# mhrice/RemFx

Hardware: AMD Instinct MI355X
Metric: audio-seconds/sec fwd+bwd (whole job) (higher is better)
Workload: dtype bf16 (fp32 accumulate); 1 GPU; Hybrid Demucs (cfg/model/demucs.yaml) train step, +exp=chorus_aug model=demucs; clips_per_gpu=64, global_batch=64, clip_samples=262144, parallelism=dp1, rccl_ranks=0, ranks=1, streams=4

## Files before the change

### include/remfx_hip.h

```cpp
#ifndef REMFX_HIP_H
#define REMFX_HIP_H

#include <stdint.h>

#ifdef __cplusplus
extern "C" {
#endif

#define RFX_ABI_VERSION 1

enum rfx_act {
  RFX_ACT_NONE = 0,
  RFX_ACT_RELU = 1,
  RFX_ACT_GELU = 2,
  RFX_ACT_TANH = 3,
  RFX_ACT_PRELU = 4,
  RFX_ACT_LEAKY = 5,
  RFX_ACT_SIGMOID = 6
};

typedef struct rfx_ktab_entry {
  int32_t off;
  int32_t da;
  int32_t db;
// ... 350 lines not shown
  void* cm_out;
  int64_t cm_ns, cm_cs, cm_as;
  int32_t cm_fold;
} rfx_cl_conv_desc;
int rfx_cl_conv(const rfx_cl_conv_desc* d, void* stream);
int rfx_cl_conv_variant(const rfx_cl_conv_desc* d);
int rfx_cl_pack(const float* src, const int32_t* idx, int64_t n, void* dst, void* stream);
int rfx_cl_from_cm(const void* src, int32_t src_bf16, int64_t s_ns, int64_t s_cs, int64_t s_as, int32_t N, int32_t C, int32_t A,
                   int32_t B, const rfx_cl_tensor* dst, const rfx_cl_tensor* res, const rfx_cl_tensor* aux, int32_t mode, void* stream);
int rfx_cl_to_cm(const rfx_cl_tensor* src, int32_t N, int32_t C, int32_t A, int32_t B, void* dst, int32_t dst_bf16, int64_t d_ns,
                 int64_t d_cs, int64_t d_as, const void* aux16, void* stream);
int rfx_cl_im2col_s4(const float* src, int64_t s_ns, int64_t s_cs, int64_t s_as, int32_t N, int32_t Cs, int32_t IA, int32_t IB, int32_t OA,
                     int32_t OB, int32_t along_b, void* dst, void* stream);
int rfx_cl_im2col_fm(const float* src, const float* coef_a, const float* coef_b, int32_t N, int32_t F, int32_t bins, void* dst, void* stream);
int rfx_fm_cm_affine(const float* in, float* out, const float* coef_a, const float* coef_b, int32_t N, int32_t bins, int32_t F, int32_t to_fm,
                     void* stream);
int rfx_cl_dgelu(const void* g, const void* z, void* out, int64_t n, void* stream);
int rfx_cl_dglu(const void* g, const void* zab, void* out, int64_t npos, int32_t C, void* stream);

typedef struct rfx_cl_wgrad_desc {
  rfx_cl_tensor p, q;
  int32_t N, OA, IA, B;
  int32_t SA, da0, NTR;
  int32_t NTC, db0, db_step;
  int32_t M, Cq, CW;
  int32_t RW, WK;
  int32_t S, ahead, bias;
  int32_t PW;
  float* ws;
} rfx_cl_wgrad_desc;
int64_t rfx_cl_wgrad_ws_floats(const rfx_cl_wgrad_desc* d);
int rfx_cl_wgrad(const rfx_cl_wgrad_desc* d, void* stream);
int rfx_cl_wgrad_variant(const rfx_cl_wgrad_desc* d);
int rfx_cl_wgrad_reduce(const float* ws, const int32_t* map, int64_t nmap, int32_t S, int32_t DT, int32_t RW, int32_t WK, float* dw,
                        int64_t wn, float* db, int32_t accumulate, void* stream);

typedef struct rfx_cl_dconv_desc {
  const void* x;
  const void* gy;
  void* y;
  void* a; void* hpre; float* stats;
  void* dz; void* dh; float* partial;
  const void* w1p; const void* w2p; const void* w2dp; const void* w1dp;
  const float *b1, *g1w, *g1b, *b2, *g2w, *g2b, *scale;
  int32_t S, C, H, dil, grid, x_or_gy_ok;
  float eps;
  int32_t TPS;
  float* tsum; float* sums;
  float* pg_dst[5];
} rfx_cl_dconv_desc;
int rfx_cl_dconv_ok(int32_t C, int32_t H, int32_t T, int32_t backward);
int rfx_cl_dconv_fwd(const rfx_cl_dconv_desc* d, void* stream);
int rfx_cl_dconv_bwd(const rfx_cl_dconv_desc* d, float* pgrad, void* stream);

int rfx_cl_rowsum(const rfx_cl_tensor* x, int32_t N, int32_t A, int32_t B, int32_t C, int32_t G, float scale, float* partial, float* out,
                  int32_t accumulate, void* stream);

int rfx_segment_split(const float* x, float* out, int32_t rows, int64_t T, int32_t L, int32_t hop, int32_t S, void* stream);
int rfx_segment_merge(const float* y, float* out, int32_t rows, int64_t T, int32_t L, int32_t hop, int32_t lead, int32_t trail,
                      int32_t S, void* stream);
int rfx_segment_split_c(const float* x, float* out, int32_t B, int32_t C, int64_t T, int32_t L, int32_t hop, int32_t S, void* stream);
int rfx_segment_merge_c(const float* y, float* out, int32_t B, int32_t Co, int64_t T, int32_t L, int32_t hop, int32_t lead, int32_t trail,
                        int32_t S, void* stream);

int rfx_fir_same(const float* x, float* y, const float* x2, float* y2, int32_t R, int64_t L, int64_t x_stride, int64_t y_stride,
                 int64_t x2_stride, int64_t y2_stride, const float* h, int32_t K, int32_t flip, void* stream);
// ... 12 lines not shown
```

### remfx_amd/_lib.py

```python
import ctypes as C
import glob
import os
import subprocess

_HERE = os.path.dirname(os.path.abspath(__file__))
_ROOT = os.path.dirname(_HERE)
CSRC = os.path.join(_HERE, "csrc")
INCLUDE = os.path.join(_ROOT, "include")
LIBDIR = os.path.join(_HERE, "_C")
LIBPATH = os.environ.get("RFX_LIBPATH_DEV") or os.path.join(LIBDIR, "libremfx_hip.so")

HIPCC_FLAGS = ["--offload-arch=gfx950", "-O3", "-std=c++17", "-fPIC", "-ffp-contract=fast",
               "-I" + INCLUDE, "-I" + CSRC]


def sources():
    return sorted(glob.glob(os.path.join(CSRC, "*.hip")))


def _stale():
    if not os.path.exists(LIBPATH):
        return True
    t = os.path.getmtime(LIBPATH)
    deps = sources() + glob.glob(os.path.join(CSRC, "*.h")) + glob.glob(os.path.join(INCLUDE, "*.h"))
# ... 53 lines not shown

class StftDesc(C.Structure):
    _fields_ = [(n, C.c_int32) for n in ("R", "T", "n_fft", "hop", "win", "bins", "frame0", "frames_out",
                                         "mode", "extra_pad_l", "extra_pad_r", "in_mode", "in_offset",
                                         "herm")] + \
               [(n, C.c_float) for n in ("scale", "eps", "alpha")] + [("accum", C.c_int32)]


class ClTensor(C.Structure):
    _fields_ = [("p", C.c_void_p), ("ns", C.c_int64), ("as_", C.c_int64), ("bs", C.c_int32), ("c0", C.c_int32)]


class ClConvDesc(C.Structure):
    _fields_ = [("inp", ClTensor)] + \
               [(n, C.c_int32) for n in ("N", "IA", "IB", "OA", "OB", "SA", "NTR", "NCH", "NTC", "KS", "da0", "da_step", "db0",
                                         "db_step", "wrapb")] + \
               [("apack", C.c_void_p)] + \
               [(n, C.c_int32) for n in ("M", "BM", "mode", "G", "g_off", "OAo", "Co")] + \
               [("bias", C.c_void_p), ("rowadd", C.c_void_p), ("out0", ClTensor), ("out1", ClTensor), ("aux0", ClTensor), ("res", ClTensor),
                ("cm_out", C.c_void_p), ("cm_ns", C.c_int64), ("cm_cs", C.c_int64), ("cm_as", C.c_int64), ("cm_fold", C.c_int32)]


class ClDconvDesc(C.Structure):
    _fields_ = [(n, C.c_void_p) for n in ("x", "gy", "y", "a", "hpre", "stats", "dz", "dh", "partial", "w1p", "w2p", "w2dp", "w1dp",
                                          "b1", "g1w", "g1b", "b2", "g2w", "g2b", "scale")] + \
               [(n, C.c_int32) for n in ("S", "C", "H", "dil", "grid", "x_or_gy_ok")] + [("eps", C.c_float), ("TPS", C.c_int32), ("tsum", C.c_void_p), ("sums", C.c_void_p), ("pg_dst", C.c_void_p * 5)]


class ClWgradDesc(C.Structure):
    _fields_ = [("p", ClTensor), ("q", ClTensor)] + \
               [(n, C.c_int32) for n in ("N", "OA", "IA", "B", "SA", "da0", "NTR", "NTC", "db0", "db_step", "M", "Cq", "CW", "RW", "WK",
                                         "S", "ahead", "bias", "PW")] + \
               [("ws", C.c_void_p)]


_P, _I32, _I64 = C.c_void_p, C.c_int32, C.c_int64
SIGNATURES = {
    "rfx_abi_version": [],
    "rfx_gemm_pick_r": [_I32, _I32],
    "rfx_pack_a": [_P, _P, _I64, _I32, _I32, _I32, _I32, _I32, _P, _P],
    "rfx_unpack_add": [_P, _P, _I64, _I32, _I32, _I32, _P, _I32, _P],
    "rfx_unpack_add_bias": [_P, _P, _I64, _I32, _I32, _I32, _P, _I32, _P, _I32, _P],
    "rfx_unpack_set": [_P, _P, _I64, _I32, _I32, _I32, _P, _I32, _P],
    "rfx_unpack_col": [_P, _I32, _I32, _I32, _I32, _P, _P],
    "rfx_gemm_fwd": [C.POINTER(GemmDesc), _P, _P, _P, _P, C.POINTER(Epilogue), _P, _P, _I32, _I32, _P, _I32, _P],
    "rfx_gemm_fwd_variant": [C.POINTER(GemmDesc), C.POINTER(Epilogue), _I32, _I32],
    "rfx_gemm_wgrad": [C.POINTER(GemmDesc), _P, _P, _P, _P, _I64, C.POINTER(C.c_int32), _I32, _P],
    "rfx_gemm_wgrad_variant": [C.POINTER(GemmDesc), _I64, _I32],
    "rfx_fft_analysis": [C.POINTER(StftDesc), _P, _P, _P, _P, _P],
    "rfx_fft_synthesis_ws": [C.POINTER(StftDesc)],
    "rfx_fft_synthesis": [C.POINTER(StftDesc), _P, _P, _P, _P, _P, _P],
    "rfx_stft_loss_reduce": [_P, _P, _I32, _I64, C.c_float, _P, _P, _P],
    "rfx_stft_loss_grad": [_P, _P, _I32, _I64, C.c_float, _P, C.c_float, C.c_float, _P, _P, _P],
    "rfx_stft_loss_grad_m": [_P, _P, _I32, _I64, C.c_float, _P, C.c_float, C.c_float, _P, _P, _P],
    "rfx_stft_pair_loss_ws": [C.POINTER(StftDesc)],
    "rfx_stft_pair_loss": [C.POINTER(StftDesc), _P, _P, _P, C.c_float, _P, _P, _P, _P, _P],
    "rfx_fft_synthesis_lossgrad": [C.POINTER(StftDesc), _P, _P, _P, C.c_float, C.c_float, C.c_float, _P, _P, _P, _P, _P],
    "rfx_l1_grad": [_P, _P, _I64, C.c_float, _P, _P, _P],
    "rfx_sisdr_sums": [_P, _P, _I32, _I64, _I64, _I64, _P, _P, _P],
    "rfx_sisdr_finish": [_P, _I32, _I64, _I32, C.c_double, _P, _P],
    "rfx_time_sums_ws": [_I32, _I64],
    "rfx_time_sums": [_P, _P, _I32, _I64, _I64, _I64, _I32, C.c_double, C.c_double, C.c_double, _P, _P, _P],
    "rfx_time_loss_rows": [_P, _I32, _I64, _I32, _I32, C.c_double, _I32, _P, _P, _P, _P],
    "rfx_time_loss_grad": [_P, _P, _I32, _I64, _I64, _I64, _P, _I32, C.c_double, C.c_double, C.c_double, _P, _I32, _P, _P],
    "rfx_logcosh_ws": [_I32, _I64],
    "rfx_logcosh_rows": [_P, _P, _I32, _I64, _I64, _I64, C.c_double, C.c_double, _P, _P, _P],
# ... 70 lines not shown
    "rfx_localstate_gen_fwd": [_P, _P, _P, _P, _I32, _I32, _I32, _I32, _I32, _P, _P, _P],
    "rfx_localstate_gen_bwd": [_P, _P, _P, _P, _P, _P, _P, _I32, _I32, _I32, _I32, _I32, _P, _P, _P, _P, _P],
    "rfx_mha_fwd": [_P, _P, _P, _I32, _I32, _I32, _I32, _P, _P, _P],
    "rfx_mha_bwd": [_P, _P, _P, _P, _P, _P, _I32, _I32, _I32, _I32, _P, _P, _P, _P],
    "rfx_localstate_mfma_ok": [_I32, _I32, _I32, _I32, _I32],
    "rfx_localstate_mfma_fwd": [_P, _P, _P, _P, _I32, _I32, _I32, _I32, _I32, _P, _P],
    "rfx_localstate_mfma_bwd": [_P, _P, _P, _P, _P, _I32, _I32, _I32, _I32, _I32, _P, _P, _P, _P, _P, _P],
    "rfx_blstm_frames": [_P, _P, _P, _I32, _I32, _I32, _I32, _I32, _I32, _I32, _P],
    "rfx_span_mask": [_P, _I32, _I32, _I32, _P, _P, _P, _P, _P],
    "rfx_dropout": [_P, _P, _I64, C.c_float, C.c_uint64, _P],
    "rfx_row_moments_slots": [_I64],
    "rfx_row_moments": [_P, _I32, _I64, _P, _P, _P, C.c_float, _P, _P, _P],
    "rfx_row_affine": [_P, _P, _P, _P, _I32, _I64, _P],
    "rfx_row_affine_add": [_P, _P, _P, _P, _P, _I32, _I32, _I64, _P],
    "rfx_fm_cm_affine_g": [_P, _P, _P, _P, _I32, _I32, _I32, _I32, _I32, _P],
    "rfx_lstm_pack_bytes": [_I32],
    "rfx_lstm_pack": [_P, _I32, _P, _P],
    "rfx_lstm_cat_params": [_P, _P, _P, _P, _P, _P, _I32, _I32, _P, _P, _P],
    "rfx_lstm_grad_scatter": [_P, _P, _I32, _I32, _P, _P, _P, _P, _P, _P, _P],
    "rfx_lstm_local": [_I32, _I32, _I32, _I32],
    "rfx_lstm_pack_local": [_P, _I32, _P, _P],
    "rfx_lstm_ws_bytes": [_I32],
    "rfx_lstm_fwd": [_P, _P, _I32, _I32, _I32, _P, _P, _P, _P, _I32, _P],
    "rfx_lstm_bwd": [_P, _P, _P, _P, _I32, _I32, _I32, _P, _P, _I32, _P],
    "rfx_lstm_set_local": [_I32, _I32],
    "rfx_channel_sum_ws": [_P, _I32, _I32, _I32, _I32, _I64, _I64, _I64, _I64],
    "rfx_channel_sum": [_P, _I32, _I32, _I32, _I32, _I64, _I64, _I64, _I64, _P, _P, _P],
    "rfx_cl_conv": [C.POINTER(ClConvDesc), _P],
    "rfx_cl_conv_variant": [C.POINTER(ClConvDesc)],
    "rfx_cl_pack": [_P, _P, _I64, _P, _P],
    "rfx_cl_wgrad_ws_floats": [_P],
    "rfx_cl_wgrad": [_P, _P],
    "rfx_cl_wgrad_variant": [_P],
    "rfx_cl_wgrad_reduce": [_P, _P, _I64, _I32, _I32, _I32, _I32, _P, _I64, _P, _I32, _P],
    "rfx_cl_from_cm": [_P, _I32, _I64, _I64, _I64, _I32, _I32, _I32, _I32, C.POINTER(ClTensor), C.POINTER(ClTensor), C.POINTER(ClTensor),
                       _I32, _P],
    "rfx_cl_rowsum": [C.POINTER(ClTensor), _I32, _I32, _I32, _I32, _I32, C.c_float, _P, _P, _I32, _P],
    "rfx_cl_to_cm": [C.POINTER(ClTensor), _I32, _I32, _I32, _I32, _P, _I32, _I64, _I64, _I64, _P, _P],
    "rfx_cl_dgelu": [_P, _P, _P, _I64, _P],
    "rfx_cl_dglu": [_P, _P, _P, _I64, _I32, _P],
    "rfx_cl_im2col_s4": [_P, _I64, _I64, _I64, _I32, _I32, _I32, _I32, _I32, _I32, _I32, _P, _P],
    "rfx_cl_im2col_fm": [_P, _P, _P, _I32, _I32, _I32, _P, _P],
    "rfx_fm_cm_affine": [_P, _P, _P, _P, _I32, _I32, _I32, _I32, _P],
    "rfx_cl_dconv_ok": [_I32, _I32, _I32, _I32],
    "rfx_cl_dconv_fwd": [_P, _P],
    "rfx_cl_dconv_bwd": [_P, _P, _P],
    "rfx_segment_split": [_P, _P, _I32, _I64, _I32, _I32, _I32, _P],
    "rfx_segment_merge": [_P, _P, _I32, _I64, _I32, _I32, _I32, _I32, _I32, _P],
    "rfx_segment_split_c": [_P, _P, _I32, _I32, _I64, _I32, _I32, _I32, _P],
    "rfx_segment_merge_c": [_P, _P, _I32, _I32, _I64, _I32, _I32, _I32, _I32, _I32, _P],
    "rfx_fir_same": [_P, _P, _P, _P, _I32, _I64, _I64, _I64, _I64, _I64, _P, _I32, _I32, _P],
    "rfx_sum_diff": [_P, _P, _P, _P, _P, _P, _I32, _I64, _I64, _I64, _I64, _I64, _P],
    "rfx_sum_diff_adj": [_P, _P, _P, _I32, _I64, _P],
}

_RET64 = {"rfx_cl_wgrad_ws_floats", "rfx_cplx_slots", "rfx_norm_bwd_work_floats", "rfx_stft_pair_loss_ws", "rfx_stft_scaled_loss_ws", "rfx_channel_sum_ws", "rfx_fft_synthesis_ws",
          "rfx_fx_phaser_ws_floats", "rfx_fx_sox_reverb_ws_floats", "rfx_fx_normalize_ws_bytes", "rfx_time_sums_ws", "rfx_logcosh_ws"}
_lib = None


def lib():
    global _lib
    if _lib is not None:
        return _lib
    import torch
    if not os.path.exists(LIBPATH):
# ... 18 lines not shown
```

### remfx_amd/clast.py

```python
import ctypes as C
import os as _os

import numpy as np
import torch

from . import _lib, ops
from ._lib import ClConvDesc, ClTensor, ClWgradDesc, check

TRACE = None

EPI = {"store": 0, "gelu": 1, "glu": 2, "dgelu": 3, "dglu": 4, "store_cm": 5}


def _stream():
    return C.c_void_p(ops.raw_stream())


def cl_tensor(t, c0=0):
    ct = ClTensor()
    if t is None:
        return ct
    if t.dtype != torch.bfloat16 or t.dim() != 4 or t.stride(3) != 1 or not t.is_cuda:
        raise ValueError(f"channels-last operand must be a 4-D bf16 GPU tensor with dense channels (got {t.dtype}, {tuple(t.shape)}, {t.stride()})")
    ct.p = t.data_ptr()
# ... 303 lines not shown
            if tiles > 16:
                continue
            ctn = -(-Cq // CW)
            cost = (ctn, ctn * CW - Cq)
            if best is None or cost < best[0]:
                best = (cost, CW, tiles)
        if best is None:
            raise ValueError(f"channels-last weight gradient: no tiling for {T} taps x {Cq} channels")
        _, self.CW, tiles = best
        self.WK = 1 if tiles > 8 else (2 if tiles > 4 else 4)
        self.WC = 8 // self.WK
        self.MTn, self.CTn = -(-M // (32 * self.RW)), -(-Cq // self.CW)
        self.DT = self.MTn * self.CTn
        hb = max(abs(db0 + t * db_step) for t in range(NTC))
        self.ahead = None
        for PW, amin in (((128, 2), (64, 1)) if _os.environ.get("RFX_CLW_PW", "128") == "128" else ((64, 1),)):
            NP = PW // 16 * self.RW
            NQ = -(-((PW + 2 * hb) * self.CW * 2) // 1024)
            PPW = -(-(NP + SA * NQ) // 8)
            if PPW > 6 or (PW // 16) % self.WK:
                continue
            for ahead in (4, 3, 2, 1):
                R = -(-(NTR + ahead * SA) // SA) * SA
                if ahead >= amin and (ahead + 1) * NP * 1024 + R * NQ * 1024 <= self.LDS_MAX and (ahead - 1) * PPW <= 24:
                    self.ahead, self.PW = ahead, PW
                    break
            if self.ahead is not None:
                break
        if self.ahead is None:
            raise ValueError("channels-last weight gradient: tile does not fit LDS")
        self.map = self._build_map(widx)
        self._dev = {}

    def _build_map(self, widx):
        RW, NT, WC = self.RW, 2, self.WC
        NCG = self.CW // 16
        HN = self.NTR * self.NTC * NCG
        bias_tile = -(-HN // 2)
        shape = (self.MTn, self.CTn, WC, RW, NT, 16, 64)
        mt, ct, cw, i, t, r, lane = np.meshgrid(*[np.arange(s, dtype=np.int64) for s in shape], indexing="ij", sparse=True)
        m = mt * 32 * RW + 32 * i + (r & 3) + 8 * (r >> 2) + 4 * (lane >> 5)
        l31 = lane & 31
        tile = cw * NT + t
        hh = 2 * tile + (l31 >> 4)
        cgl, tt = hh % NCG, hh // NCG
        tc, tr = tt % self.NTC, tt // self.NTC
        c = ct * self.CW + cgl * 16 + (l31 & 15)
        ok = (hh < HN) & (m < self.M) & (c < self.Cq)
        idx = widx(np.minimum(m, self.M - 1), np.minimum(tr, self.NTR - 1), tc, np.minimum(c, self.Cq - 1))
        out = np.where(np.broadcast_to(ok, shape), np.broadcast_to(idx, shape), -1)
        if self.bias:
            isb = (tile == bias_tile) & (l31 == 0) & (ct == 0) & (m < self.M)
            out = np.where(np.broadcast_to(isb, shape), np.broadcast_to(self.wn + m, shape), out)
        flat = out.reshape(-1)
        used = flat[flat >= 0]
        assert used.size == np.unique(used).size, "weight-gradient map: a destination is written twice"
        return np.ascontiguousarray(flat.astype(np.int32))

    def splits(self, steps):
        S = max(1, min(steps, -(-CLW_SPLITS // self.DT)))
        sps = -(-steps // S)
        return -(-steps // sps)


def _dev_map(form, device):
    key = str(device)
    v = form._dev.get(key)
    if v is None:
        v = torch.from_numpy(form.map).to(device)
        form._dev[key] = v
    return v


def wgrad(form, p, q, N, OA, IA, B, dw, db=None, accumulate=False, p_c0=0, q_c0=0):
    if form.bias and db is None:
        raise ValueError("this weight-gradient form carries the bias gradient: pass db")
    d = ClWgradDesc()
    d.p, d.q = cl_tensor(p, p_c0), cl_tensor(q, q_c0)
    d.N, d.OA, d.IA, d.B = N, OA, IA, B
# ... 54 lines not shown
```

### remfx_amd/csrc/cl_wgrad.hip

```cpp
#include "cl_common.h"

#ifndef RFX_CLW_DBG_BUILD
#define RFX_CLW_DBG_BUILD 0
#endif
#define CLW_DBG RFX_CLW_DBG_BUILD
#include <stdlib.h>

struct ClWgK {
  rfx_cl_wgrad_desc d;
  int32_t nbq, MTn, CTn, DT, spx;
  int32_t total, sps;
  int32_t NP, NQ, TP, PPW;
  int32_t PSLOT, QROWB, QROWP, R, PD, PRE, HB;
  int32_t HN, NCG, bias_tile;
  uint32_t p_bytes, q_bytes;
};

#define CL_WG_MAXP 6

__device__ __forceinline__ void clw_wait_vm(int n) {
  switch (n) {
    case 0: CL_VMCNT(0); break;   case 1: CL_VMCNT(1); break;   case 2: CL_VMCNT(2); break;   case 3: CL_VMCNT(3); break;
    case 4: CL_VMCNT(4); break;   case 5: CL_VMCNT(5); break;   case 6: CL_VMCNT(6); break;   case 7: CL_VMCNT(7); break;
    case 8: CL_VMCNT(8); break;   case 9: CL_VMCNT(9); break;   case 10: CL_VMCNT(10); break; case 11: CL_VMCNT(11); break;
    case 12: CL_VMCNT(12); break; case 13: CL_VMCNT(13); break; case 14: CL_VMCNT(14); break; case 15: CL_VMCNT(15); break;
    case 16: CL_VMCNT(16); break; case 17: CL_VMCNT(17); break; case 18: CL_VMCNT(18); break; case 19: CL_VMCNT(19); break;
    case 20: CL_VMCNT(20); break; case 21: CL_VMCNT(21); break; case 22: CL_VMCNT(22); break; case 23: CL_VMCNT(23); break;
    default: CL_VMCNT(24); break;
  }
}

typedef short clw_s16x4 __attribute__((ext_vector_type(4)));
typedef short clw_s16x8 __attribute__((ext_vector_type(8)));
__device__ __forceinline__ cl_bf16x8 clw_frag(const unsigned char* p, int step4) {
  const clw_s16x4 lo = __builtin_amdgcn_ds_read_tr16_b64_v4i16((__attribute__((address_space(3))) clw_s16x4*)(p));
  const clw_s16x4 hi = __builtin_amdgcn_ds_read_tr16_b64_v4i16((__attribute__((address_space(3))) clw_s16x4*)(p + step4));
  const clw_s16x8 v = {lo[0], lo[1], lo[2], lo[3], hi[0], hi[1], hi[2], hi[3]};
  return __builtin_bit_cast(cl_bf16x8, v);
}

struct ClwIt {
  int n, bq, oa, pre;
};

template <int RW, int WK, int PW>
__global__ __launch_bounds__(512, 2) void cl_wgrad_kernel(const ClWgK g) {
  constexpr int NT = 2, WC = 8 / WK, KSW = (PW / 16) / WK;
  constexpr int PROWB = 64 * RW;
  extern __shared__ __attribute__((aligned(16))) unsigned char clw_smem[];
  const rfx_cl_wgrad_desc& d = g.d;
  const int tid = threadIdx.x;
  const int wave = __builtin_amdgcn_readfirstlane(tid >> 6), lane = tid & 63;
  const int kq = wave / WC, cw = wave % WC;
  const int bid = blockIdx.x, xcd = bid & 7, qx = bid >> 3;
  const bool grouped = d.S >= 8;
  const int dt = grouped ? qx % g.DT : bid % g.DT, split = grouped ? xcd * g.spx + qx / g.DT : bid / g.DT;
  if (split >= d.S) return;
  const int mt = dt / g.CTn, ct = dt - mt * g.CTn;
  const int tau0 = split * g.sps;
  const int tau1 = min(tau0 + g.sps, g.total);
  const int OA = d.OA;

  unsigned char* const pbase_lds = clw_smem;
  unsigned char* const qbase_lds = clw_smem + g.PD * g.PSLOT;

  int32_t rel[CL_WG_MAXP], bpos[CL_WG_MAXP];
  int lds_off[CL_WG_MAXP], prow[CL_WG_MAXP];
#pragma unroll
  for (int i = 0; i < CL_WG_MAXP; ++i) {
    int e = wave + 8 * i;
    e = e < g.TP ? e : g.TP - 1;
    if (e < g.NP) {
      prow[i] = -1;
      lds_off[i] = e * 1024;
      const int o = e * 1024 + lane * 16;
      const int pos = o / PROWB, cb = o - pos * PROWB;
      const bool ok = pos < PW && (mt * 32 * RW + (cb >> 1)) < d.M;
      rel[i] = ok ? (int32_t)((pos * d.p.bs + d.p.c0 + mt * 32 * RW) * 2 + cb) : (int32_t)CL_OOB;
      bpos[i] = 0;
    } else {
      const int qe = e - g.NP;
      const int rr = qe / g.NQ, qi = qe - rr * g.NQ;
      prow[i] = rr;
      lds_off[i] = rr * g.QROWB + qi * 1024;
      const int o = qi * 1024 + lane * 16;
      const int pos = o / g.QROWP, cb = o - pos * g.QROWP;
      const bool ok = pos < PW + 2 * g.HB && (ct * d.CW + (cb >> 1)) < d.Cq;
      rel[i] = ok ? (int32_t)(((pos - g.HB) * d.q.bs + d.q.c0 + ct * d.CW) * 2 + cb) : (int32_t)CL_OOB;
      bpos[i] = ok ? pos - g.HB : 0x40000000;
    }
  }

  const int gq = lane >> 4, i16 = lane & 15;
  const int rowhalf = gq & 1, khalf = gq >> 1, s_e = i16 >> 2, q4 = i16 & 3;
  const uint32_t a0 = (uint32_t)((8 * khalf + s_e) * PROWB + rowhalf * 32 + q4 * 8);
  int rtap[NT];
  uint32_t bconst[NT];
#pragma unroll
  for (int t = 0; t < NT; ++t) {
    int hh = 2 * (cw * NT + t) + rowhalf;
    hh = hh < g.HN ? hh : 0;
    const int cgl = hh % g.NCG, tt = hh / g.NCG;
    const int tc = tt % d.NTC;
    rtap[t] = tt / d.NTC;
    bconst[t] = (uint32_t)((g.HB + d.db0 + tc * d.db_step + 8 * khalf + s_e) * g.QROWP + cgl * 32 + q4 * 8);
  }
  const bool ones_wave = d.bias && g.bias_tile >= 0 && (g.bias_tile / NT) == cw;
  const int ones_t = g.bias_tile % NT;

  f32x16 acc[RW][NT];
#pragma unroll
  for (int i = 0; i < RW; ++i)
#pragma unroll
    for (int t = 0; t < NT; ++t)
#pragma unroll
      for (int r = 0; r < 16; ++r) acc[i][t][r] = 0.f;

  const int col0 = tau0 / OA;
  const int ncols = (tau1 - 1) / OA - col0 + 1;
  const int L = (tau1 - tau0) + g.PRE * ncols;
  ClwIt it_i = {col0 / g.nbq, col0 % g.nbq, tau0 - col0 * OA - g.PRE, g.PRE}, it_c = it_i;
  auto advance = [&](ClwIt& it) {
    ++it.oa;
    if (it.pre > 0) --it.pre;
    if (it.oa == OA) {
      it.oa = -g.PRE; it.pre = g.PRE;
      if (++it.bq == g.nbq) { it.bq = 0; ++it.n; }
    }
  };
  int rs_n = it_i.n;
  cl_i32x4 rs_p = cl_rsrc_words(reinterpret_cast<const uint16_t*>(d.p.p) + (int64_t)rs_n * d.p.ns, g.p_bytes);
  cl_i32x4 rs_q = cl_rsrc_words(reinterpret_cast<const uint16_t*>(d.q.p) + (int64_t)rs_n * d.q.ns, g.q_bytes);
  int iu = 0, wp = 0, ps_i = 0;
  auto issue_next = [&]() {
    if (CLW_DBG & 1) { advance(it_i); ++iu; return; }
    const int b0 = it_i.bq * PW;
    const bool real = it_i.pre == 0;
    if (it_i.n != rs_n) {
// ... 4 lines not shown
    const int32_t pb = (int32_t)(((int64_t)it_i.oa * d.p.as + (int64_t)b0 * d.p.bs) * 2);
    const int ia0 = it_i.oa * d.SA + d.da0 + d.NTR - d.SA;
#pragma unroll
    for (int i = 0; i < CL_WG_MAXP; ++i) {
      if (i < g.PPW) {
        if (prow[i] < 0) {
          const uint32_t vo = real ? (uint32_t)(rel[i] + pb) : CL_OOB;
          cl_glds16_quiet(rs_p, pbase_lds + ps_i * g.PSLOT + lds_off[i], vo);
        } else {
          const int ia = ia0 + prow[i];
          const bool rok = (unsigned)ia < (unsigned)d.IA;
          const int32_t qb = (int32_t)(((int64_t)ia * d.q.as + (int64_t)b0 * d.q.bs) * 2);
          const uint32_t vo = (rok && (unsigned)(b0 + bpos[i]) < (unsigned)d.B) ? (uint32_t)(rel[i] + qb) : CL_OOB;
          cl_glds16_quiet(rs_q, qbase_lds + wp * g.QROWB + lds_off[i], vo);
        }
      }
    }
    wp += d.SA;
    wp = wp >= g.R ? wp - g.R : wp;
    ps_i = ps_i + 1 == g.PD ? 0 : ps_i + 1;
    advance(it_i);
    ++iu;
  };

  int cpm = (d.SA - d.NTR + 2 * g.R) % g.R;
  int ps_c = 0;
  const int ahead = g.PD - 1;
  for (int i = 0; i < ahead; ++i)
    if (iu < L) issue_next();
  const bool late = wave >= 4 && !(CLW_DBG & 16);
  auto frags = [&](int ks, const unsigned char* pb, const unsigned char* const (&qb)[NT], cl_bf16x8 (&af)[RW], cl_bf16x8 (&bf)[NT], int i) {
#pragma unroll
    for (int r = 0; r < RW; ++r)
      af[r] = (CLW_DBG & 2) ? __builtin_bit_cast(cl_bf16x8, make_uint4(lane, r, ks, i)) : clw_frag(pb + ks * 16 * PROWB + r * 64, 4 * PROWB);
#pragma unroll
    for (int t = 0; t < NT; ++t) {
      if (ones_wave && t == ones_t) {
        const clw_s16x8 one = {0x3f80, 0x3f80, 0x3f80, 0x3f80, 0x3f80, 0x3f80, 0x3f80, 0x3f80};
        bf[t] = __builtin_bit_cast(cl_bf16x8, one);
      } else {
        bf[t] = (CLW_DBG & 2) ? __builtin_bit_cast(cl_bf16x8, make_uint4(lane, t, ks, i)) : clw_frag(qb[t] + ks * 16 * g.QROWP, 4 * g.QROWP);
      }
    }
  };
  for (int i = 0; i < L; ++i) {
    const int left = L - 1 - i;
    clw_wait_vm((left < ahead - 1 ? left : ahead - 1) * g.PPW);
    if (!(CLW_DBG & 8)) __builtin_amdgcn_s_barrier();
    __builtin_amdgcn_sched_barrier(0);
    if (!late && iu < L) issue_next();
    __builtin_amdgcn_sched_barrier(0);
    if (it_c.pre == 0 && !(CLW_DBG & 4)) {
      const unsigned char* pb = pbase_lds + ps_c * g.PSLOT + a0;
      const unsigned char* qb[NT];
#pragma unroll
      for (int t = 0; t < NT; ++t) {
        int sl = cpm + rtap[t];
        sl = sl >= g.R ? sl - g.R : sl;
        qb[t] = qbase_lds + sl * g.QROWB + bconst[t];
      }
      cl_bf16x8 af[2][RW], bf[2][NT];
      frags(kq, pb, qb, af[0], bf[0], i);
#pragma unroll
      for (int ksi = 0; ksi < KSW; ++ksi) {
        if (ksi + 1 < KSW) frags(kq + (ksi + 1) * WK, pb, qb, af[(ksi + 1) & 1], bf[(ksi + 1) & 1], i);
#pragma unroll
        for (int r = 0; r < RW; ++r)
#pragma unroll
          for (int t = 0; t < NT; ++t) acc[r][t] = __builtin_amdgcn_mfma_f32_32x32x16_bf16(af[ksi & 1][r], bf[ksi & 1][t], acc[r][t], 0, 0, 0);
      }
    }
    __builtin_amdgcn_sched_barrier(0);
    if (late && iu < L) issue_next();
    cpm += d.SA;
    cpm = cpm >= g.R ? cpm - g.R : cpm;
    ps_c = ps_c + 1 == g.PD ? 0 : ps_c + 1;
    advance(it_c);
  }

  float* wsp = d.ws + ((size_t)((size_t)split * g.DT + dt) * 8 + wave) * (RW * NT * 16 * 64) + lane;
#pragma unroll
  for (int r = 0; r < RW; ++r)
#pragma unroll
    for (int t = 0; t < NT; ++t)
#pragma unroll
      for (int e = 0; e < 16; ++e) wsp[((r * NT + t) * 16 + e) * 64] = acc[r][t][e];
// ... 12 lines not shown
    hb = v < 0 ? (-v > hb ? -v : hb) : (v > hb ? v : hb);
  }
  if (hb > 8) return -1;
  k.d = d;
  k.HB = hb;
  k.nbq = d.B / d.PW;
  k.MTn = (d.M + 32 * d.RW - 1) / (32 * d.RW);
  k.CTn = (d.Cq + d.CW - 1) / d.CW;
  k.DT = k.MTn * k.CTn;
  k.spx = (d.S + 7) / 8;
  const int64_t total = (int64_t)d.N * k.nbq * d.OA;
  if (total >= 0x7fffffffLL) return -1;
  k.total = (int)total;
  k.sps = (int)((total + d.S - 1) / d.S);
  if ((total + k.sps - 1) / k.sps != d.S) return -1;
  k.NCG = d.CW / 16;
  k.HN = d.NTR * d.NTC * k.NCG;
  const int WC = 8 / d.WK, tiles = (k.HN + 1) / 2;
  if (tiles > WC * 2) return -1;
  k.bias_tile = d.bias ? tiles : -1;
  if (d.bias && tiles + 1 > WC * 2) return -1;
  k.NP = (d.PW * 64 * d.RW + 1023) / 1024;
  k.QROWP = d.CW * 2;
  k.NQ = ((d.PW + 2 * hb) * k.QROWP + 1023) / 1024;
  k.TP = k.NP + d.SA * k.NQ;
  k.PPW = (k.TP + 7) / 8;
  if (k.PPW > CL_WG_MAXP) return -1;
  k.PSLOT = k.NP * 1024;
  k.QROWB = k.NQ * 1024;
  k.PRE = (d.NTR - d.SA + d.SA - 1) / d.SA;
  k.PD = d.ahead + 1;
  k.R = ((d.NTR + d.ahead * d.SA + d.SA - 1) / d.SA) * d.SA;
  if ((k.PD - 2) * k.PPW > 24 && k.PD > 2) return -1;
  const int64_t pb = ((int64_t)(d.OA - 1) * d.p.as + (int64_t)d.B * d.p.bs) * 2;
  const int64_t qb = ((int64_t)(d.IA - 1) * d.q.as + (int64_t)d.B * d.q.bs) * 2;
  if (pb <= 0 || qb <= 0 || pb >= 0x7fffffffLL || qb >= 0x7fffffffLL) return -1;
  k.p_bytes = (uint32_t)pb;
  k.q_bytes = (uint32_t)qb;
  return 0;
}

template <int RW, int WK, int PW>
static int clw_launch1(const ClWgK& k, int lds, hipStream_t s, bool query) {
  const bool grouped = k.d.S >= 8;
  if (query) return RW | WK << 2 | PW << 5 | (grouped ? 1 : 0) << 13;
  static int attr_lds = 0;
  if (lds > attr_lds) {
    if (hipFuncSetAttribute(reinterpret_cast<const void*>(&cl_wgrad_kernel<RW, WK, PW>), hipFuncAttributeMaxDynamicSharedMemorySize, lds) !=
        hipSuccess)
      return -3;
    attr_lds = lds;
  }
  hipLaunchKernelGGL((cl_wgrad_kernel<RW, WK, PW>), dim3((unsigned)(grouped ? 8 * k.spx * k.DT : k.d.S * k.DT)), dim3(512), lds, s, k);
  RFX_CHECK_LAUNCH();
  return 0;
}
template <int RW, int WK>
static int clw_launch(const ClWgK& k, int lds, hipStream_t s, bool query) {
  return k.d.PW == 128 ? clw_launch1<RW, WK, 128>(k, lds, s, query) : clw_launch1<RW, WK, 64>(k, lds, s, query);
}

extern "C" int64_t rfx_cl_wgrad_ws_floats(const rfx_cl_wgrad_desc* dp) {
  ClWgK k;
  if (!dp || clw_geometry(*dp, k)) return -1;
  return (int64_t)dp->S * k.DT * 8 * dp->RW * 2 * 1024;
}

static int clw_run(const rfx_cl_wgrad_desc* dp, void* stream, bool query) {
  if (!dp || !dp->p.p || !dp->q.p || !dp->ws) return -1;
  ClWgK k;
  if (clw_geometry(*dp, k)) return -1;
  const int lds = k.PD * k.PSLOT + k.R * k.QROWB;
  if (lds > 160 * 1024) return -1;
  hipStream_t s = (hipStream_t)stream;
  if (dp->RW == 3) {
    if (dp->WK == 1) return clw_launch<3, 1>(k, lds, s, query);
    if (dp->WK == 2) return clw_launch<3, 2>(k, lds, s, query);
    return clw_launch<3, 4>(k, lds, s, query);
  }
  if (dp->WK == 1) return clw_launch<2, 1>(k, lds, s, query);
  if (dp->WK == 2) return clw_launch<2, 2>(k, lds, s, query);
  return clw_launch<2, 4>(k, lds, s, query);
}
extern "C" int rfx_cl_wgrad(const rfx_cl_wgrad_desc* dp, void* stream) { return clw_run(dp, stream, false); }
extern "C" int rfx_cl_wgrad_variant(const rfx_cl_wgrad_desc* dp) { return clw_run(dp, nullptr, true); }

__global__ __launch_bounds__(256) void cl_wgrad_reduce_kernel(const float* __restrict__ ws, const int32_t* __restrict__ map, int64_t nmap,
                                                              int S, int DT, int WC, int WK, int per_wave, float* __restrict__ dw,
                                                              int64_t wn, float* __restrict__ db, int accumulate) {
  __shared__ float part[4][64];
  const int l = threadIdx.x & 63, sg = threadIdx.x >> 6;
  const int64_t e = (int64_t)blockIdx.x * 64 + l;
  const int32_t dst = e < nmap ? map[e] : -1;
  float sum = 0.f;
  if (dst >= 0) {
    const int64_t inner = e % per_wave;
    const int64_t dc = e / per_wave;
    const int cw = (int)(dc % WC);
    const int64_t dt = dc / WC;
    const int nsrc = S * WK;
    const int per = (nsrc + 3) / 4;
    const int i0 = sg * per, i1 = min(i0 + per, nsrc);
    const int64_t sstride = (int64_t)DT * 8 * per_wave;
    const float* base = ws + dt * 8 * per_wave + (int64_t)cw * per_wave + inner;
    auto src = [&](int i) { return base[(int64_t)(i / WK) * sstride + (int64_t)(i % WK) * WC * per_wave]; };
    int i = i0;
    for (; i + 8 <= i1; i += 8) {
      float v[8];
#pragma unroll
      for (int u = 0; u < 8; ++u) v[u] = src(i + u);
#pragma unroll
      for (int u = 0; u < 8; ++u) sum += v[u];
    }
    for (; i < i1; ++i) sum += src(i);
  }
  part[sg][l] = sum;
  __syncthreads();
  if (sg == 0 && dst >= 0) {
// ... 17 lines not shown
```

Measured before the change: 3742 audio-seconds/sec.

## Swizzle wgrad LDS layouts and reorder 48-channel tile enumeration to cut bank conflicts

Changes the LDS layout of the channels-last weight-gradient kernel. P rows are XOR-swizzled for RW=2, and Q rows get a 64-channel XOR swizzle or a blocked 48-channel layout with per-row flipping. A custom half-tile enumeration table is used for CW=48, NTC=3, with the matching host-side map in Python. The aim is fewer LDS bank conflicts in the MFMA fragment loads. A layout query API is added for verification, and the extra address arithmetic plus the Python/device mapping consistency are added risks.

```diff
diff --git a/include/remfx_hip.h b/include/remfx_hip.h
--- a/include/remfx_hip.h
+++ b/include/remfx_hip.h
@@ -406,6 +406,14 @@
 int64_t rfx_cl_wgrad_ws_floats(const rfx_cl_wgrad_desc* d);
 int rfx_cl_wgrad(const rfx_cl_wgrad_desc* d, void* stream);
 int rfx_cl_wgrad_variant(const rfx_cl_wgrad_desc* d);
+typedef struct rfx_cl_wgrad_lane {
+  int32_t a_addr[3][2];
+  int32_t b_addr[2][2], b_half[2], b_cg[2], b_tc[2], b_tr[2], b_row[2];
+  int32_t dma_row, dma_addr, dma_pos, dma_ch, dma_zero;
+  int32_t p_slot_bytes, q_row_bytes, q_rows, pieces, halo;
+} rfx_cl_wgrad_lane;
+int rfx_cl_wgrad_layout(const rfx_cl_wgrad_desc* d, int32_t dt, int32_t wave, int32_t lane, int32_t ks, int32_t piece,
+                        rfx_cl_wgrad_lane* out);
 int rfx_cl_wgrad_reduce(const float* ws, const int32_t* map, int64_t nmap, int32_t S, int32_t DT, int32_t RW, int32_t WK, float* dw,
                         int64_t wn, float* db, int32_t accumulate, void* stream);
 
diff --git a/remfx_amd/_lib.py b/remfx_amd/_lib.py
--- a/remfx_amd/_lib.py
+++ b/remfx_amd/_lib.py
@@ -109,6 +109,13 @@
                [(n, C.c_int32) for n in ("N", "OA", "IA", "B", "SA", "da0", "NTR", "NTC", "db0", "db_step", "M", "Cq", "CW", "RW", "WK",
                                          "S", "ahead", "bias", "PW")] + \
                [("ws", C.c_void_p)]
+
+
+class ClWgradLane(C.Structure):
+    _fields_ = [("a_addr", (C.c_int32 * 2) * 3), ("b_addr", (C.c_int32 * 2) * 2)] + \
+               [(n, C.c_int32 * 2) for n in ("b_half", "b_cg", "b_tc", "b_tr", "b_row")] + \
+               [(n, C.c_int32) for n in ("dma_row", "dma_addr", "dma_pos", "dma_ch", "dma_zero", "p_slot_bytes", "q_row_bytes", "q_rows",
+                                         "pieces", "halo")]
 
 
 _P, _I32, _I64 = C.c_void_p, C.c_int32, C.c_int64
@@ -245,6 +252,7 @@
     "rfx_cl_wgrad_ws_floats": [_P],
     "rfx_cl_wgrad": [_P, _P],
     "rfx_cl_wgrad_variant": [_P],
+    "rfx_cl_wgrad_layout": [_P, _I32, _I32, _I32, _I32, _I32, _P],
     "rfx_cl_wgrad_reduce": [_P, _P, _I64, _I32, _I32, _I32, _I32, _P, _I64, _P, _I32, _P],
     "rfx_cl_from_cm": [_P, _I32, _I64, _I64, _I64, _I32, _I32, _I32, _I32, C.POINTER(ClTensor), C.POINTER(ClTensor), C.POINTER(ClTensor),
                        _I32, _P],
diff --git a/remfx_amd/clast.py b/remfx_amd/clast.py
--- a/remfx_amd/clast.py
+++ b/remfx_amd/clast.py
@@ -359,6 +359,19 @@
         self.map = self._build_map(widx)
         self._dev = {}
 
+    HALF9 = (((0, 0), (0, 1), (1, 0), (1, 1), (2, 0), (2, 1), (0, 2), (1, 2), (2, 2)),
+             ((2, 1), (0, 0), (0, 1), (1, 1), (1, 2), (1, 0), (2, 0), (0, 2), (2, 2)))
+
+    def half(self, hh):
+        NCG = self.CW // 16
+        if self.CW == 48 and self.NTC == 3:
+            tab = np.array(self.HALF9, dtype=np.int64)
+            tr, i = hh // 9, hh % 9
+            e = tab[tr & 1, i]
+            return e[..., 1], e[..., 0], tr
+        cgl, tt = hh % NCG, hh // NCG
+        return cgl, tt % self.NTC, tt // self.NTC
+
     def _build_map(self, widx):
         RW, NT, WC = self.RW, 2, self.WC
         NCG = self.CW // 16
@@ -370,8 +383,7 @@
         l31 = lane & 31
         tile = cw * NT + t
         hh = 2 * tile + (l31 >> 4)
-        cgl, tt = hh % NCG, hh // NCG
-        tc, tr = tt % self.NTC, tt // self.NTC
+        cgl, tc, tr = self.half(hh)
         c = ct * self.CW + cgl * 16 + (l31 & 15)
         ok = (hh < HN) & (m < self.M) & (c < self.Cq)
         idx = widx(np.minimum(m, self.M - 1), np.minimum(tr, self.NTR - 1), tc, np.minimum(c, self.Cq - 1))
diff --git a/remfx_amd/csrc/cl_wgrad.hip b/remfx_amd/csrc/cl_wgrad.hip
--- a/remfx_amd/csrc/cl_wgrad.hip
+++ b/remfx_amd/csrc/cl_wgrad.hip
@@ -4,6 +4,7 @@
 #define RFX_CLW_DBG_BUILD 0
 #endif
 #define CLW_DBG RFX_CLW_DBG_BUILD
+#define CLW_IDENT ((CLW_DBG & 32) != 0)
 #include <stdlib.h>
 
 struct ClWgK {
@@ -13,8 +14,114 @@
   int32_t NP, NQ, TP, PPW;
   int32_t PSLOT, QROWB, QROWP, R, PD, PRE, HB;
   int32_t HN, NCG, bias_tile;
+  int32_t QL, QFLIP, ENUM9;
   uint32_t p_bytes, q_bytes;
 };
+
+enum { CLW_QL_ROWS = 0, CLW_QL_X64 = 1, CLW_QL_B48 = 2 };
+
+template <int RW>
+__host__ __device__ __forceinline__ int clw_p_off(int pos, int ch) {
+  if (RW == 2 && !CLW_IDENT) ch ^= (pos & 2) << 1;
+  return pos * (64 * RW) + (ch << 4);
+}
+template <int RW>
+__host__ __device__ __forceinline__ void clw_p_at(int o, int& pos, int& ch) {
+  pos = o / (64 * RW);
+  ch = (o - pos * (64 * RW)) >> 4;
+  if (RW == 2 && !CLW_IDENT) ch ^= (pos & 2) << 1;
+}
+__host__ __device__ __forceinline__ int clw_q_off(int ql, int rowp, int x, int ch, int flip) {
+  if (ql == CLW_QL_X64) return x * 128 + ((ch ^ ((x & 2) << 1)) << 4);
+  if (ql == CLW_QL_B48) return (x >> 3) * 768 + (((((x >> 2) & 1) ^ flip) * 24 + (ch >> 1) * 8 + (x & 3) * 2 + (ch & 1)) << 4);
+  return x * rowp + (ch << 4);
+}
+__host__ __device__ __forceinline__ void clw_q_at(int ql, int rowp, int o, int flip, int& x, int& ch) {
+  if (ql == CLW_QL_B48) {
+    const int blk = o / 768;
+    int k = (o - blk * 768) >> 4;
+    const int w = k / 24;
+    k -= w * 24;
+    x = blk * 8 + ((w ^ flip) << 2) + ((k & 7) >> 1);
+    ch = (k >> 3) * 2 + (k & 1);
+    return;
+  }
+  x = o / rowp;
+  ch = (o - x * rowp) >> 4;
+  if (ql == CLW_QL_X64) ch ^= (x & 2) << 1;
+}
+
+__host__ __device__ __forceinline__ void clw_half(const ClWgK& g, int hh, int& cgl, int& tc, int& tr) {
+  if (g.ENUM9) {
+    tr = hh / 9;
+    const unsigned long long tab = (tr & 1) ? 0xA28465109ull : 0xA62985410ull;
+    const int v = (int)(tab >> (4 * (hh - tr * 9))) & 15;
+    cgl = v & 3;
+    tc = v >> 2;
+    return;
+  }
+  cgl = hh % g.NCG;
+  const int tt = hh / g.NCG;
+  tc = tt % g.d.NTC;
+  tr = tt / g.d.NTC;
+}
+
+struct ClwPiece {
+  int prow, lds_off;
+  int pos, cb;
+  bool ok;
+};
+template <int RW>
+__host__ __device__ __forceinline__ ClwPiece clw_piece(const ClWgK& g, int mt, int ct, int wave, int lane, int i) {
+  const rfx_cl_wgrad_desc& d = g.d;
+  ClwPiece r;
+  int e = wave + 8 * i, ch;
+  e = e < g.TP ? e : g.TP - 1;
+  if (e < g.NP) {
+    r.prow = -1;
+    r.lds_off = e * 1024;
+    clw_p_at<RW>(e * 1024 + lane * 16, r.pos, ch);
+    r.cb = ch << 4;
+    r.ok = r.pos < d.PW && (mt * 32 * RW + (r.cb >> 1)) < d.M;
+  } else {
+    const int qe = e - g.NP;
+    const int rr = qe / g.NQ, qi = qe - rr * g.NQ;
+    r.prow = rr;
+    r.lds_off = rr * g.QROWB + qi * 1024;
+    clw_q_at(g.QL, g.QROWP, qi * 1024 + lane * 16, g.QFLIP & rr & 1, r.pos, ch);
+    r.cb = ch << 4;
+    r.ok = r.pos < d.PW + 2 * g.HB && (ct * d.CW + (r.cb >> 1)) < d.Cq;
+  }
+  return r;
+}
+
+template <int RW>
+__host__ __device__ __forceinline__ void clw_a_addr(int lane, uint32_t (&a)[RW]) {
+  const int gq = lane >> 4, i16 = lane & 15;
+  const int rowhalf = gq & 1, khalf = gq >> 1, s_e = i16 >> 2, q4 = i16 & 3;
+#pragma unroll
+  for (int r = 0; r < RW; ++r) a[r] = (uint32_t)(clw_p_off<RW>(8 * khalf + s_e, r * 4 + rowhalf * 2 + (q4 >> 1)) + (q4 & 1) * 8);
+}
+struct ClwB {
+  int hh, cgl, tc, tr, flip;
+  uint32_t lo;
+  int32_t hi;
+};
+__host__ __device__ __forceinline__ ClwB clw_b_addr(const ClWgK& g, int cw, int t, int lane) {
+  const rfx_cl_wgrad_desc& d = g.d;
+  const int gq = lane >> 4, i16 = lane & 15;
+  const int rowhalf = gq & 1, khalf = gq >> 1, s_e = i16 >> 2, q4 = i16 & 3;
+  ClwB b;
+  b.hh = 2 * (cw * 2 + t) + rowhalf;
+  b.hh = b.hh < g.HN ? b.hh : g.HN - 1;
+  clw_half(g, b.hh, b.cgl, b.tc, b.tr);
+  const int cpm0 = (d.SA - d.NTR + 2 * g.R) % g.R;
+  b.flip = g.QFLIP & (cpm0 + b.tr) & 1;
+  const int x = g.HB + d.db0 + b.tc * d.db_step + 8 * khalf + s_e, ch = b.cgl * 2 + (q4 >> 1);
+  b.lo = (uint32_t)(clw_q_off(g.QL, g.QROWP, x, ch, b.flip) + (q4 & 1) * 8);
+  b.hi = clw_q_off(g.QL, g.QROWP, x + 4, ch, b.flip) + (q4 & 1) * 8 - (int32_t)b.lo;
+  return b;
+}
 
 #define CL_WG_MAXP 6
 
@@ -68,42 +175,29 @@
   int lds_off[CL_WG_MAXP], prow[CL_WG_MAXP];
 #pragma unroll
   for (int i = 0; i < CL_WG_MAXP; ++i) {
-    int e = wave + 8 * i;
-    e = e < g.TP ? e : g.TP - 1;
-    if (e < g.NP) {
-      prow[i] = -1;
-      lds_off[i] = e * 1024;
-      const int o = e * 1024 + lane * 16;
-      const int pos = o / PROWB, cb = o - pos * PROWB;
-      const bool ok = pos < PW && (mt * 32 * RW + (cb >> 1)) < d.M;
-      rel[i] = ok ? (int32_t)((pos * d.p.bs + d.p.c0 + mt * 32 * RW) * 2 + cb) : (int32_t)CL_OOB;
+    const ClwPiece pc = clw_piece<RW>(g, mt, ct, wave, lane, i);
+    prow[i] = pc.prow;
+    lds_off[i] = pc.lds_off;
+    if (pc.prow < 0) {
+      rel[i] = pc.ok ? (int32_t)((pc.pos * d.p.bs + d.p.c0 + mt * 32 * RW) * 2 + pc.cb) : (int32_t)CL_OOB;
       bpos[i] = 0;
     } else {
-      const int qe = e - g.NP;
-      const int rr = qe / g.NQ, qi = qe - rr * g.NQ;
-      prow[i] = rr;
-      lds_off[i] = rr * g.QROWB + qi * 1024;
-      const int o = qi * 1024 + lane * 16;
-      const int pos = o / g.QROWP, cb = o - pos * g.QROWP;
-      const bool ok = pos < PW + 2 * g.HB && (ct * d.CW + (cb >> 1)) < d.Cq;
-      rel[i] = ok ? (int32_t)(((pos - g.HB) * d.q.bs + d.q.c0 + ct * d.CW) * 2 + cb) : (int32_t)CL_OOB;
-      bpos[i] = ok ? pos - g.HB : 0x40000000;
-    }
-  }
-
-  const int gq = lane >> 4, i16 = lane & 15;
-  const int rowhalf = gq & 1, khalf = gq >> 1, s_e = i16 >> 2, q4 = i16 & 3;
-  const uint32_t a0 = (uint32_t)((8 * khalf + s_e) * PROWB + rowhalf * 32 + q4 * 8);
+      rel[i] = pc.ok ? (int32_t)(((pc.pos - g.HB) * d.q.bs + d.q.c0 + ct * d.CW) * 2 + pc.cb) : (int32_t)CL_OOB;
+      bpos[i] = pc.ok ? pc.pos - g.HB : 0x40000000;
+    }
+  }
+
+  uint32_t a0[RW];
+  clw_a_addr<RW>(lane, a0);
   int rtap[NT];
   uint32_t bconst[NT];
+  int32_t bhi[NT];
 #pragma unroll
   for (int t = 0; t < NT; ++t) {
-    int hh = 2 * (cw * NT + t) + rowhalf;
-    hh = hh < g.HN ? hh : 0;
-    const int cgl = hh % g.NCG, tt = hh / g.NCG;
-    const int tc = tt % d.NTC;
-    rtap[t] = tt / d.NTC;
-    bconst[t] = (uint32_t)((g.HB + d.db0 + tc * d.db_step + 8 * khalf + s_e) * g.QROWP + cgl * 32 + q4 * 8);
+    const ClwB b = clw_b_addr(g, cw, t, lane);
+    rtap[t] = b.tr;
+    bconst[t] = b.lo;
+    bhi[t] = b.hi;
   }
   const bool ones_wave = d.bias && g.bias_tile >= 0 && (g.bias_tile / NT) == cw;
   const int ones_t = g.bias_tile % NT;
@@ -174,14 +268,14 @@
   auto frags = [&](int ks, const unsigned char* pb, const unsigned char* const (&qb)[NT], cl_bf16x8 (&af)[RW], cl_bf16x8 (&bf)[NT], int i) {
 #pragma unroll
     for (int r = 0; r < RW; ++r)
-      af[r] = (CLW_DBG & 2) ? __builtin_bit_cast(cl_bf16x8, make_uint4(lane, r, ks, i)) : clw_frag(pb + ks * 16 * PROWB + r * 64, 4 * PROWB);
+      af[r] = (CLW_DBG & 2) ? __builtin_bit_cast(cl_bf16x8, make_uint4(lane, r, ks, i)) : clw_frag(pb + a0[r] + ks * 16 * PROWB, 4 * PROWB);
 #pragma unroll
     for (int t = 0; t < NT; ++t) {
       if (ones_wave && t == ones_t) {
         const clw_s16x8 one = {0x3f80, 0x3f80, 0x3f80, 0x3f80, 0x3f80, 0x3f80, 0x3f80, 0x3f80};
         bf[t] = __builtin_bit_cast(cl_bf16x8, one);
       } else {
-        bf[t] = (CLW_DBG & 2) ? __builtin_bit_cast(cl_bf16x8, make_uint4(lane, t, ks, i)) : clw_frag(qb[t] + ks * 16 * g.QROWP, 4 * g.QROWP);
+        bf[t] = (CLW_DBG & 2) ? __builtin_bit_cast(cl_bf16x8, make_uint4(lane, t, ks, i)) : clw_frag(qb[t] + ks * 16 * g.QROWP, bhi[t]);
       }
     }
   };
@@ -193,7 +287,7 @@
     if (!late && iu < L) issue_next();
     __builtin_amdgcn_sched_barrier(0);
     if (it_c.pre == 0 && !(CLW_DBG & 4)) {
-      const unsigned char* pb = pbase_lds + ps_c * g.PSLOT + a0;
+      const unsigned char* pb = pbase_lds + ps_c * g.PSLOT;
       const unsigned char* qb[NT];
 #pragma unroll
       for (int t = 0; t < NT; ++t) {
@@ -272,6 +366,9 @@
   k.PD = d.ahead + 1;
   k.R = ((d.NTR + d.ahead * d.SA + d.SA - 1) / d.SA) * d.SA;
   if ((k.PD - 2) * k.PPW > 24 && k.PD > 2) return -1;
+  k.QL = CLW_IDENT ? CLW_QL_ROWS : d.CW == 64 ? CLW_QL_X64 : (d.CW == 48 && ((d.PW + 2 * hb + 7) / 8) * 768 <= k.QROWB) ? CLW_QL_B48 : CLW_QL_ROWS;
+  k.QFLIP = k.QL == CLW_QL_B48 && d.SA % 2 == 0;
+  k.ENUM9 = d.CW == 48 && d.NTC == 3;
   const int64_t pb = ((int64_t)(d.OA - 1) * d.p.as + (int64_t)d.B * d.p.bs) * 2;
   const int64_t qb = ((int64_t)(d.IA - 1) * d.q.as + (int64_t)d.B * d.q.bs) * 2;
   if (pb <= 0 || qb <= 0 || pb >= 0x7fffffffLL || qb >= 0x7fffffffLL) return -1;
@@ -324,6 +421,44 @@
 }
 extern "C" int rfx_cl_wgrad(const rfx_cl_wgrad_desc* dp, void* stream) { return clw_run(dp, stream, false); }
 extern "C" int rfx_cl_wgrad_variant(const rfx_cl_wgrad_desc* dp) { return clw_run(dp, nullptr, true); }
+
+template <int RW>
+static void clw_view(const ClWgK& k, int dt, int wave, int lane, int ks, int piece, rfx_cl_wgrad_lane* o) {
+  const rfx_cl_wgrad_desc& d = k.d;
+  const int WC = 8 / d.WK, cw = wave % WC, mt = dt / k.CTn, ct = dt - mt * k.CTn;
+  uint32_t a[RW];
+  clw_a_addr<RW>(lane, a);
+  for (int r = 0; r < 3; ++r)
+    for (int h = 0; h < 2; ++h) o->a_addr[r][h] = r < RW ? (int32_t)a[r] + (ks * 16 + h * 4) * 64 * RW : -1;
+  const bool ones_wave = d.bias && k.bias_tile >= 0 && (k.bias_tile / 2) == cw;
+  const int cpm0 = (d.SA - d.NTR + 2 * k.R) % k.R;
+  for (int t = 0; t < 2; ++t) {
+    const ClwB b = clw_b_addr(k, cw, t, lane);
+    const bool ones = ones_wave && t == k.bias_tile % 2;
+    const bool live = 2 * (cw * 2 + t) + ((lane >> 4) & 1) < k.HN;
+    o->b_half[t] = ones ? -1 : live ? b.hh : -2;
+    o->b_cg[t] = b.cgl, o->b_tc[t] = b.tc, o->b_tr[t] = b.tr;
+    o->b_row[t] = (cpm0 + b.tr) % k.R;
+    o->b_addr[t][0] = (int32_t)b.lo + ks * 16 * k.QROWP;
+    o->b_addr[t][1] = o->b_addr[t][0] + b.hi;
+  }
+  o->p_slot_bytes = k.PSLOT, o->q_row_bytes = k.QROWB, o->q_rows = k.R, o->pieces = k.PPW, o->halo = k.HB;
+  const ClwPiece pc = clw_piece<RW>(k, mt, ct, wave, lane, piece);
+  o->dma_row = pc.prow < 0 ? -1 : pc.prow;
+  o->dma_addr = (pc.prow < 0 ? pc.lds_off : pc.lds_off - pc.prow * k.QROWB) + lane * 16;
+  o->dma_zero = !pc.ok;
+  o->dma_pos = pc.prow < 0 ? pc.pos : pc.pos - k.HB;
+  o->dma_ch = pc.cb >> 1;
+}
+extern "C" int rfx_cl_wgrad_layout(const rfx_cl_wgrad_desc* dp, int32_t dt, int32_t wave, int32_t lane, int32_t ks, int32_t piece,
+                                   rfx_cl_wgrad_lane* out) {
+  ClWgK k;
+  if (!dp || !out || clw_geometry(*dp, k)) return -1;
+  if (dt < 0 || dt >= k.DT || wave < 0 || wave > 7 || lane < 0 || lane > 63 || ks < 0 || ks >= dp->PW / 16 || piece < 0 || piece >= k.PPW) return -1;
+  if (dp->RW == 3) clw_view<3>(k, dt, wave, lane, ks, piece, out);
+  else clw_view<2>(k, dt, wave, lane, ks, piece, out);
+  return 0;
+}
 
 __global__ __launch_bounds__(256) void cl_wgrad_reduce_kernel(const float* __restrict__ ws, const int32_t* __restrict__ map, int64_t nmap,
                                                               int S, int DT, int WC, int WK, int per_wave, float* __restrict__ dw,
```

After: 3741 audio-seconds/sec. Within noise of the previous version (-0.0%).
